# ethereum/pos-evolution

Measured on AMD Instinct MI355X. Metric: attestations aggregated/sec + get_head() p50 latency at 1M validators, higher is better.
Workload: dtype int32

## Files before the change

### pos_evolution_amd/csrc/engine_g1.cpp

```cpp
#include "engine_internal.h"

using namespace posevo;

namespace posevo {

void g1_stream_guard(pe_engine* h, hipStream_t s)
{
    if (h->side_ever && s != h->side_stream && s != h->fin_stream && s != h->norm_stream) (void)hipStreamWaitEvent(s, h->ev_join, 0);
}

int build_points30(pe_engine* h, uint64_t n)
{
    HIP_TRY(h, h->d_points30.ensure(std::max<size_t>(128, 4ull * G1_ROW_WORDS * n)));
    launch_g1_table_s30(h->stream, h->d_points.as<uint32_t>(), h->d_points30.as<uint32_t>(), n);
    HIP_TRY(h, hipGetLastError());
    h->points30_valid = true;
    return PE_OK;
}

int launch_g1_planned(pe_engine* h, const uint32_t* d_points, const uint32_t* d_members, const uint32_t* d_bits,
                      const G1Group* d_groups, const G1Plan& plan, uint8_t* d_out96, uint32_t* dev_jac,
                      hipStream_t s, hipStream_t fin, DevBuf* partials, DevBuf* lane_partials, const AttPlan* plan_dev,
                      const uint32_t* d_members1, uint64_t caller_rows, const G1Complement* cm)
{
    if (plan.n_groups == 0) return PE_OK;
    if (!s) s = h->stream;
    if (!fin) fin = s;
    if (!partials) partials = &h->d_partials;
    if (!lane_partials) lane_partials = &h->d_lane_partials;
    PE_TRY(ensure_quiesced(h, *partials,
                           std::max<size_t>(PE_G1_PARTIAL_BYTES, (size_t)PE_G1_PARTIAL_BYTES * plan.n_partials)));
    const size_t lane_bytes = (size_t)G1_LANE_PARTIAL_BYTES * G1_WG * ((plan.n_slots + G1_WG - 1) / G1_WG);
    PE_TRY(ensure_quiesced(h, *lane_partials, std::max<size_t>(PE_G1_PARTIAL_BYTES, lane_bytes)));
    const uint32_t* d_points30;
    if (d_points == h->d_points.as<uint32_t>()) {
        if (!h->points30_valid) return fail(h, PE_ERR_STATE, "the registry's table of the accumulation's field form was not built");
        d_points30 = h->d_points30.as<uint32_t>();
    } else {
        const uint64_t n_rows = caller_rows;
        if (d_points != h->d_tmp_points.as<uint32_t>() || 4ull * G1_ROW_WORDS * n_rows > h->d_tmp_points.cap)
            return fail(h, PE_ERR_STATE, "G1 sum over an unknown point table");
        HIP_TRY(h, h->d_tmp_points30.ensure(std::max<size_t>(128, 4ull * G1_ROW_WORDS * n_rows)));
        launch_g1_table_s30(s, d_points, h->d_tmp_points30.as<uint32_t>(), n_rows);
        d_points30 = h->d_tmp_points30.as<uint32_t>();
    }
    const bool chain = fin != s && fin == h->fin_stream;
    const int exclusive = chain && h->tune.exclusive && h->blocks.size() <= 4096 ? 1 : 0;
    const uint32_t sparse_max = cm && cm->info ? h->tune.g1_sparse_max() : 0u;
    const uint32_t* sparse_info = sparse_max ? cm->info : nullptr;
    if (sparse_max)
        launch_g1_absentees(s, d_points30, d_members, d_members1, d_bits, d_groups, plan.n_groups, plan_dev, cm->cmpl, sparse_info,
                            sparse_max, partials->as<uint32_t>());
    {
        const bool skip = !h->prof_timeline && s != h->stream && (h->acc_launches++ & 3) != 0;
        ProfScope ps(h, PE_KERNEL_G1_ACCUMULATE, s, skip);
        unsigned long long* clock_rec = nullptr;
        if (h->profiling) {
            if (!h->acc_clock && hipHostMalloc(reinterpret_cast<void**>(&h->acc_clock), 16ull * pe_engine::ACC_CLOCK_RING,
                                               hipHostMallocDefault) != hipSuccess) {
                (void)hipGetLastError();
                h->acc_clock = nullptr;
            }
            if (h->acc_clock) {
                clock_rec = h->acc_clock + 2 * (h->acc_clock_n++ % pe_engine::ACC_CLOCK_RING);
                clock_rec[0] = clock_rec[1] = 0;
            }
        }
        launch_g1_accumulate(s, d_points30, d_members, d_bits, d_groups, plan.n_groups, plan.n_slots,
                             lane_partials->as<uint32_t>(), partials->as<uint32_t>(), plan_dev, d_members1, exclusive, clock_rec,
                             cm ? cm->cmpl : nullptr, sparse_info, sparse_max);
    }
    hipStream_t ts = fin;
    if (ts != s) {
        HIP_TRY(h, hipEventRecord(h->ev_acc, s));
        HIP_TRY(h, hipStreamWaitEvent(ts, h->ev_acc, 0));
    }
    {
        ProfScope ps(h, PE_KERNEL_G1_TREE, ts);
        launch_g1_tree(ts, lane_partials->as<uint32_t>(), d_groups, plan.n_groups, plan.n_slots, partials->as<uint32_t>(),
                       ts != s ? 1 : 0,
                       plan_dev, exclusive, sparse_max ? cm->cmpl : nullptr, sparse_info, sparse_max);
    }
    hipStream_t ns = fin;
    if (chain && h->norm_stream) {
        ns = h->norm_stream;
        HIP_TRY(h, hipEventRecord(h->ev_tree, ts));
        HIP_TRY(h, hipStreamWaitEvent(ns, h->ev_tree, 0));
    } else if (ts != fin) {
        HIP_TRY(h, hipEventRecord(h->ev_tree, ts));
        HIP_TRY(h, hipStreamWaitEvent(fin, h->ev_tree, 0));
    }
    if (cm)
        for (int t = 0; t < 2; ++t)
            if (cm->ev[t]) HIP_TRY(h, hipStreamWaitEvent(ns, cm->ev[t], 0));
    {
        ProfScope ps(h, PE_KERNEL_G1_NORMALISE, ns);
        launch_g1_finish(ns, partials->as<uint32_t>(), d_groups, plan.n_groups, 0, 0, d_out96, dev_jac, plan_dev,
                         cm ? cm->cmpl : nullptr, cm ? cm->sums[0] : nullptr, cm ? cm->sums[1] : nullptr);
    }
    HIP_TRY(h, hipGetLastError());
    return PE_OK;
}

void committee_sums_drop(pe_engine* h)
{
    for (auto& t : h->tables) t.sums_valid = t.sums_wanted = false;
    if (h->sums_stream) (void)hipStreamSynchronize(h->sums_stream);
}
int build_committee_sums(pe_engine* h, CommitteeTable* t, bool defer)
{
    t->sums_valid = false;
    t->sums_wanted = false;
    if (!h->tune.committee_sums || !t->is_partition || !h->have_points || !h->points30_valid || h->dist_ready()) return PE_OK;
    if (t->n_committees == 0 || t->n_val_at_load != h->n_val || t->offsets.size() != (size_t)t->n_committees + 1) return PE_OK;
    const uint32_t C = t->n_committees;
    uint64_t total = t->offsets.back();
    uint32_t max_size = 0;
    for (uint32_t c = 0; c < C; ++c) max_size = std::max(max_size, t->offsets[c + 1] - t->offsets[c]);
    if (total == 0) return PE_OK;
    const uint32_t k = (uint32_t)std::max<uint64_t>({(uint64_t)G1_MIN_K, (total + G1_TARGET_LANES - 1) / G1_TARGET_LANES,
                                                     ((uint64_t)max_size + G1_WG - 1) / G1_WG});
    const uint32_t tasks = (max_size + k - 1) / k;
    uint32_t l2 = 0;
    while ((1u << l2) < tasks) ++l2;
    const uint64_t slots = (uint64_t)C << l2;
    if (slots > 4ull * G1_TARGET_LANES) return PE_OK;
    if (!h->sums_stream) {
        int least = 0, greatest = 0;
        HIP_TRY(h, hipDeviceGetStreamPriorityRange(&least, &greatest));
        HIP_TRY(h, hipStreamCreateWithPriority(&h->sums_stream, hipStreamNonBlocking, least));
    }
    hipStream_t ps = h->sums_stream;
    const size_t lane_bytes = (size_t)G1_LANE_PARTIAL_BYTES * G1_WG * ((slots + G1_WG - 1) / G1_WG);
    if (sizeof(G1Group) * (size_t)C > h->d_sum_groups.cap || lane_bytes > h->d_sum_lane.cap ||
        (size_t)PE_G1_PARTIAL_BYTES * C > t->d_sums.cap)
        HIP_TRY(h, hipStreamSynchronize(ps));
    HIP_TRY(h, h->d_sum_groups.ensure(sizeof(G1Group) * (size_t)C));
    HIP_TRY(h, h->d_sum_lane.ensure(lane_bytes));
    HIP_TRY(h, t->d_sums.ensure((size_t)PE_G1_PARTIAL_BYTES * C));
    if (defer) {
        t->sums_wanted = true;
        return PE_OK;
    }
    HIP_TRY(h, hipMemsetAsync(t->d_sums.p, 0, (size_t)PE_G1_PARTIAL_BYTES * C, ps));
    G1Group* d_groups = h->d_sum_groups.as<G1Group>();
    launch_g1_committee_groups(ps, t->d_offsets.as<uint32_t>(), C, k, l2, d_groups);
    launch_g1_accumulate(ps, h->d_points30.as<uint32_t>(), t->d_members.as<uint32_t>(), nullptr, d_groups, C, (uint32_t)slots,
                         h->d_sum_lane.as<uint32_t>(), t->d_sums.as<uint32_t>());
    launch_g1_tree(ps, h->d_sum_lane.as<uint32_t>(), d_groups, C, (uint32_t)slots, t->d_sums.as<uint32_t>());
    HIP_TRY(h, hipGetLastError());
    if (!t->ev_sums) HIP_TRY(h, hipEventCreateWithFlags(&t->ev_sums, hipEventDisableTiming));
    HIP_TRY(h, hipEventRecord(t->ev_sums, ps));
    t->sums_valid = true;
    return PE_OK;
}

int committee_sums_build_wanted(pe_engine* h, CommitteeTable* t)
{
    if (!t->sums_wanted || t->sums_valid || t->ready_pending) return PE_OK;
    if (t->ev_ready && hipEventQuery(t->ev_ready) != hipSuccess) { (void)hipGetLastError(); return PE_OK; }
    if (h->prep_stream && hipStreamQuery(h->prep_stream) != hipSuccess) { (void)hipGetLastError(); return PE_OK; }
    return build_committee_sums(h, t, false);
}

int sig_batch_flush(pe_engine* h)
{
    if (h->sig_batch.empty()) return PE_OK;
    std::vector<pe_engine::SigSeg> segs;
    segs.swap(h->sig_batch);
    const bool own = h->aux_stream && h->stream == h->own_stream;
    hipStream_t ss = own ? leg_stream(h) : h->stream;
    bool between = own && h->side_stream != nullptr;
    for (auto& sg : segs) between = between && sg.streaming;
    hipStream_t ds = between ? h->side_stream : ss;
    if (between) ss = ds;
    if (ss != h->stream) {
        HIP_TRY(h, hipEventRecord(h->ev_aux_fork, h->stream));
        HIP_TRY(h, hipStreamWaitEvent(ss, h->ev_aux_fork, 0));
        if (ds != ss) HIP_TRY(h, hipStreamWaitEvent(ds, h->ev_aux_fork, 0));
    }
    G2DecompressBatch b{};
    for (auto& sg : segs) {
        if (sg.copy_from) HIP_TRY(h, hipMemcpyAsync(const_cast<uint8_t*>(sg.d_in), sg.copy_from, sg.bytes, hipMemcpyDeviceToDevice, ds));
        if (sg.compressed) {
            b.in96[b.count] = sg.d_in;
            b.out_mont48[b.count] = sg.d_pts;
            b.status[b.count] = sg.d_status;
            b.n[b.count] = sg.n;
            ++b.count;
        } else {
            HIP_TRY(h, hipMemsetAsync(sg.d_status, 0, 4ull * sg.n, ds));
            launch_g2_convert(ds, sg.d_in, sg.d_pts, sg.n);
        }
    }
    if (b.count) {
        ProfScope ps(h, PE_KERNEL_G2_DECOMPRESS, ds);
        launch_g2_decompress_batch(ds, b);
    }
    if (ds != ss) {
        HIP_TRY(h, hipEventRecord(h->ev_sig, ds));
        HIP_TRY(h, hipStreamWaitEvent(ss, h->ev_sig, 0));
    }
    G2AggregateRowsBatch r{};
    for (auto& sg : segs) {
        if (sg.check_subgroup) launch_g2_subgroup_check(ss, sg.d_pts, sg.n, sg.d_status);
        r.pts[r.count] = sg.d_pts;
        r.status[r.count] = sg.d_status;
        r.ug[r.count] = sg.d_ug;
        r.member_row[r.count] = sg.d_member_row;
        r.plan_dev[r.count] = sg.plan_dev;
        r.out96[r.count] = sg.o_sig;
        r.out_bad[r.count] = sg.o_bad;
        r.n_groups[r.count] = sg.ng_bound;
        r.keep_mont48[r.count] = sg.keep_mont48;
        r.keep_bad[r.count] = sg.keep_bad;
        ++r.count;
    }
    {
        ProfScope ps(h, PE_KERNEL_G2_ACCUMULATE, ss);
        launch_g2_aggregate_rows(ss, r);
    }
    G2StatusOutBatch so{};
    for (auto& sg : segs) {
        so.src[so.count] = sg.d_status;
        so.dst_host[so.count] = sg.o_st;
        so.n[so.count] = sg.n;
        ++so.count;
    }
    launch_g2_status_out(ss, so);
    for (auto& sg : segs) {
        if (ss != h->stream) {
            pe_engine::PipeArena& a = h->arena[sg.arena];
            HIP_TRY(h, hipEventRecord(a.ev_leg, ss));
            a.leg_used = true;
        }
    }
    HIP_TRY(h, hipGetLastError());
    return PE_OK;
}
bool sig_batch_holds(const pe_engine* h, int arena)
{
    for (const auto& sg : h->sig_batch)
        if (sg.arena == arena) return true;
    return false;
}


int settle_signatures(pe_engine* h, const uint8_t* signatures96, uint64_t n, size_t tail_words, bool check_subgroup,
                      bool mark_identity, HostLap* lap, SettledSigs* out)
{
    hipStream_t s = h->stream;
// ... 544 lines not shown
```

### pos_evolution_amd/csrc/fp381_s30.h

```cpp
#pragma once
#include <stdint.h>

#include "pe_hd.h"

#ifndef PE_FQ30_ACC
#define PE_FQ30_ACC int64_t
#endif

namespace posevo {
namespace s30 {

constexpr int FQ_B = 30, FQ_N = 13;
constexpr int32_t FQ_MASK = (1 << FQ_B) - 1;

#include "fp381_s30_consts.inc"


using fq_acc = PE_FQ30_ACC;
PE_HD int32_t fq_digit32(int32_t v);
PE_HD int32_t fq_mont_digit(uint32_t v) { return fq_digit32((int32_t)v); }
PE_HD int32_t fq_carry32(int32_t v) { return (v >> FQ_B) + (int32_t)(((uint32_t)v >> (FQ_B - 1)) & 1u); }
PE_HD int32_t fq_norm_carry(int32_t v, int32_t) { return fq_carry32(v); }
PE_HD int32_t fq_p_carried(int i) { return FQ_P_CARRIED[i]; }

#include "fp381_lazy.inc"

PE_HD void fq_balance(fq& r, const fq& a)
{
    int32_t c = 0;
#pragma unroll
    for (int i = 0; i < FQ_N - 1; ++i) {
        const int32_t v = a.l[i] + c;
        r.l[i] = fq_digit32(v);
        c = fq_carry32(v);
    }
    r.l[FQ_N - 1] = a.l[FQ_N - 1] + c;
}
PE_HD void fq_from_mont32(fq& r, const uint32_t* w)
{
    fq a, an, k, t, c;
    fq_from_words32(a, w);
    fq_norm(an, a);
#pragma unroll
    for (int i = 0; i < FQ_N; ++i) k.l[i] = FQ_FROM_R32[i];
    fq_mul(t, an, k);
    fq_canonical_near(c, t);
    fq_balance(r, c);
}

}
}
```

### pos_evolution_amd/csrc/g1_kernels.hip

```cpp
#define POSEVO_FP_MUL_CALLED 1
#include <algorithm>
#include <hip/hip_ext.h>
#include "g1.h"
#include "g1_s30.h"
#include "fp_sqrt.h"
#include "kernels.h"
#include "wave64.h"

namespace posevo {

__global__ void __launch_bounds__(256) k_g1_convert(const uint8_t* __restrict__ be96, uint32_t* __restrict__ mont24,
                                                     uint64_t n)
{
    uint64_t i = (uint64_t)blockIdx.x * blockDim.x + threadIdx.x;
    if (i >= n) return;
    const uint8_t* src = be96 + 96 * i;
    uint32_t* dst = mont24 + (uint64_t)G1_ROW_WORDS * i;
    if (src[0] & 0x40) {
#pragma unroll
        for (int j = 0; j < 24; ++j) dst[j] = 0;
        return;
    }
    fp x, y, xm, ym;
    fp_load_be48(x, src);
// ... 694 lines not shown
        }
    }
    const bool gated = d.bits_word != NONE32;
    auto want = [&](uint32_t j, uint32_t& idx) -> bool {
        const uint32_t i = first + j;
        idx = members ? members[d.member_start + i] : d.member_start + i;
        if (!gated) return true;
        return (((bit_arena[d.bits_word + (i >> 5)] >> (i & 31)) & 1u) ^ invert) != 0;
    };
    auto fetch = [&](uint32_t j, fq& ox, fq& oy) -> bool {
        uint32_t idx;
        if (!want(j, idx)) return false;
        return load_point_s30(ox, oy, pts30, idx);
    };
    {
        fq qx, qy, nx, ny;
        bool have = false, nhave = false, w1 = false, w2 = false;
        uint32_t i1 = 0, i2 = 0;
        if (count > 0) {
            uint32_t i0;
            if (want(0, i0)) have = load_point_s30(qx, qy, pts30, i0);
        }
        if (count > 1) w1 = want(1, i1);
        for (uint32_t j = 0; j < count; ++j) {
            w2 = false;
            if (j + 2 < count) w2 = want(j + 2, i2);
            nhave = false;
            if (w1) nhave = load_point_s30(nx, ny, pts30, i1);
            if (have) {
                if (acc.inf) g1q_set_first(acc, qx, qy);
                else g1q_madd_fast(acc, qx, qy, exc);
            }
            qx = nx; qy = ny; have = nhave;
            i1 = i2; w1 = w2;
        }
    }
    G1_STAMP(1);
    G1_WAVE_END();
    if (exc) {
        g1q_set_inf(acc);
        for (uint32_t j = 0; j < count; ++j) {
            fq qx, qy;
            if (fetch(j, qx, qy)) g1q_add_affine<FqCalled>(acc, qx, qy, false);
        }
    }
    uint32_t* b = lane_partials + (size_t)blockIdx.x * G1S_WORDS * G1_WG + tid;
    const bool inf = acc.inf;
#pragma unroll
    for (int k = 0; k < FQ_N; ++k) {
        b[k * G1_WG] = inf ? 0u : (uint32_t)acc.x.l[k];
        b[(FQ_N + k) * G1_WG] = inf ? 0u : (uint32_t)acc.y.l[k];
        b[(2 * FQ_N + k) * G1_WG] = inf ? 0u : (uint32_t)acc.zz.l[k];
        b[(3 * FQ_N + k) * G1_WG] = inf ? 0u : (uint32_t)acc.zzz.l[k];
    }
    if (my_size == 1) {
        uint32_t* dst = wg_partials + (size_t)G1X_WORDS * my_out;
#pragma nounroll
        for (int c = 0; c < 4; ++c) {
            uint32_t w[12];
            fq_to_mont32_via<FqCalled>(w, acc.x);
#pragma unroll
            for (int k = 0; k < 12; ++k) dst[12 * c + k] = inf ? 0u : w[k];
            acc.x = acc.y;
            acc.y = acc.zz;
            acc.zz = acc.zzz;
        }
    }
    if (clock_rec && blockIdx.x == 0 && tid == 0) {
        clock_rec[0] = wall_clock64() - rec_w0;
        clock_rec[1] = clock64() - rec_c0;
    }
}
}

__global__ void __launch_bounds__(G1_WG) __attribute__((amdgpu_waves_per_eu(2, 2)))
k_g1_accumulate(const uint32_t* __restrict__ pts30, const uint32_t* __restrict__ members,
                const uint32_t* __restrict__ bit_arena, const G1Group* __restrict__ groups, uint32_t n_groups,
                uint32_t n_slots, uint32_t* __restrict__ lane_partials, uint32_t* __restrict__ wg_partials,
                const AttPlan* __restrict__ plan_dev, const uint32_t* __restrict__ members1,
                unsigned long long* __restrict__ clock_rec, const uint32_t* __restrict__ cmpl,
                const uint32_t* __restrict__ sparse_info, uint32_t sparse_max)
{
    s30::g1_accumulate_body(pts30, members, bit_arena, groups, n_groups, n_slots, lane_partials, wg_partials, plan_dev,
                            members1, clock_rec, cmpl, sparse_info, sparse_max);
}

void launch_g1_table_s30(hipStream_t s, const uint32_t* points_mont24, uint32_t* points_s30, uint64_t n)
{
    if (n == 0) return;
    hipLaunchKernelGGL(k_g1_table_s30, dim3((unsigned)((n + 255) / 256)), dim3(256), 0, s, points_mont24, points_s30, n);
}
void launch_g1_accumulate(hipStream_t s, const uint32_t* points_s30, const uint32_t* members,
                              const uint32_t* bit_arena, const G1Group* groups, uint32_t n_groups, uint32_t n_slots,
                              uint32_t* lane_partials, uint32_t* wg_partials48, const AttPlan* plan_dev,
                              const uint32_t* members1, int exclusive, unsigned long long* clock_rec, const uint32_t* cmpl,
                              const uint32_t* sparse_info, uint32_t sparse_max)
{
    if (n_groups == 0 || n_slots == 0) return;
    const unsigned blocks = (n_slots + G1_WG - 1) / G1_WG;
    size_t lds_bytes = 0;
    if (exclusive) {
        lds_bytes = G1_ACC_EXCLUSIVE_LDS;
        if (first_use_on_this_device<82>())
            (void)hipFuncSetAttribute(reinterpret_cast<const void*>(k_g1_accumulate), hipFuncAttributeMaxDynamicSharedMemorySize,
                                      (int)G1_ACC_EXCLUSIVE_LDS);
    }
    hipLaunchKernelGGL(k_g1_accumulate, dim3(blocks), dim3(G1_WG), lds_bytes, s, points_s30, members, bit_arena,
                       groups, n_groups, n_slots, lane_partials, wg_partials48, plan_dev, members1, clock_rec, cmpl, sparse_info,
                       sparse_max);
}

void launch_g1_tree(hipStream_t s, const uint32_t* lane_partials, const G1Group* groups, uint32_t n_groups,
                    uint32_t n_slots, uint32_t* wg_partials48, int one_per_cu, const AttPlan* plan_dev, int solo,
                    const uint32_t* cmpl, const uint32_t* sparse_info, uint32_t sparse_max)
{
    if (n_groups == 0 || n_slots == 0) return;
    const unsigned blocks = (n_slots + G1_WG - 1) / G1_WG;
    size_t lds_bytes = (s30::G1S_WORDS + 2) * G1_WG * sizeof(uint32_t);
    if (solo) {
        hipLaunchKernelGGL(k_g1_tree_solo, dim3(blocks), dim3(G1_WG), lds_bytes, s, lane_partials, groups, n_groups, n_slots,
                           wg_partials48, plan_dev, cmpl, sparse_info, sparse_max);
        return;
    }
    if (one_per_cu) {
        constexpr size_t padded = 84 * 1024;
        if (first_use_on_this_device<84>())
            (void)hipFuncSetAttribute(reinterpret_cast<const void*>(k_g1_tree), hipFuncAttributeMaxDynamicSharedMemorySize,
                                      (int)padded);
        lds_bytes = padded;
    }
    hipLaunchKernelGGL(k_g1_tree, dim3(blocks), dim3(G1_WG), lds_bytes, s, lane_partials, groups, n_groups, n_slots,
                       wg_partials48, plan_dev, cmpl, sparse_info, sparse_max);
}

namespace s30 {
__device__ __forceinline__ void g1q_from_lane_down(g1q& q, const g1q& p, int off)
{
#pragma unroll
    for (int j = 0; j < FQ_N; ++j) {
        q.x.l[j] = __shfl_down(p.x.l[j], off, 64);
        q.y.l[j] = __shfl_down(p.y.l[j], off, 64);
        q.zz.l[j] = __shfl_down(p.zz.l[j], off, 64);
        q.zzz.l[j] = __shfl_down(p.zzz.l[j], off, 64);
    }
    q.inf = __shfl_down((int)p.inf, off, 64) != 0;
    q.affine = false;
}
__device__ __forceinline__ void g1_absentees_body(const uint32_t* __restrict__ pts30, const uint32_t* __restrict__ members,
                                                  const uint32_t* __restrict__ members1,
                                                  const uint32_t* __restrict__ bit_arena, const G1Group* __restrict__ groups,
                                                  uint32_t n_groups, const AttPlan* __restrict__ plan_dev,
                                                  const uint32_t* __restrict__ cmpl,
                                                  const uint32_t* __restrict__ sparse_info, uint32_t sparse_max,
                                                  uint32_t* __restrict__ wg_partials)
{
    __shared__ uint32_t list[G1_SPARSE_CAP];
    if (plan_dev) n_groups = min(n_groups, plan_dev->n_groups);
    const uint32_t g = blockIdx.x;
    if (g >= n_groups) return;
    const G1Group d = groups[g];
    if (!g1_group_sparse(d, g, cmpl, sparse_info, sparse_max)) return;
    const uint32_t lane = threadIdx.x;
    const uint32_t n_words = (d.n_members + 31) >> 5;
    const uint32_t tail_mask = (d.n_members & 31) ? ((1u << (d.n_members & 31)) - 1u) : 0xFFFFFFFFu;
    uint32_t total = 0;
    for (uint32_t w0 = 0; w0 < n_words; w0 += 64) {
        const uint32_t w = w0 + lane;
        uint32_t absent = 0;
        if (w < n_words) absent = ~bit_arena[d.bits_word + w] & (w == n_words - 1 ? tail_mask : 0xFFFFFFFFu);
        const uint32_t mine = (uint32_t)__builtin_popcount(absent);
        uint32_t pos = total + wave_incl_scan(mine) - mine;
        while (absent) {
            if (pos < G1_SPARSE_CAP) list[pos] = 32u * w + (uint32_t)__builtin_ctz(absent);
            ++pos;
            absent &= absent - 1;
        }
        total += wave_sum(mine);
    }
    total = min(total, G1_SPARSE_CAP);
    __syncthreads();
    const uint32_t* __restrict__ mem = (d.k >> 31) ? members1 : members;
    g1q acc;
    g1q_set_inf(acc);
    for (uint32_t e = lane; e < total; e += 64) {
        const uint32_t i = list[e];
        const uint32_t idx = mem ? mem[d.member_start + i] : d.member_start + i;
        fq qx, qy;
        const bool have = load_point_s30(qx, qy, pts30, idx);
        g1q_add_affine<FqCalled>(acc, qx, qy, !have);
    }
    uint32_t live = min(total, 64u);
#pragma nounroll
    for (uint32_t off = 32; off >= 1; off >>= 1) {
        if (live <= off) continue;
        g1q q;
        g1q_from_lane_down(q, acc, (int)off);
        if (lane < off && lane + off < live) g1q_add<FqCalled>(acc, q);
        live = off;
    }
    fq coord;
#pragma unroll
    for (int j = 0; j < FQ_N; ++j) {
        const int32_t x = __shfl(acc.x.l[j], 0, 64), y = __shfl(acc.y.l[j], 0, 64);
        const int32_t zz = __shfl(acc.zz.l[j], 0, 64), zzz = __shfl(acc.zzz.l[j], 0, 64);
        coord.l[j] = lane == 0 ? x : lane == 1 ? y : lane == 2 ? zz : zzz;
    }
    const bool inf = __shfl((int)acc.inf, 0, 64) != 0;
    if (lane < 4) {
        uint32_t w[12];
        fq_to_mont32_via<FqCalled>(w, coord);
        uint4* dst = reinterpret_cast<uint4*>(wg_partials + (size_t)G1X_WORDS * d.out_base + 12 * lane);
        dst[0] = inf ? make_uint4(0, 0, 0, 0) : make_uint4(w[0], w[1], w[2], w[3]);
        dst[1] = inf ? make_uint4(0, 0, 0, 0) : make_uint4(w[4], w[5], w[6], w[7]);
        dst[2] = inf ? make_uint4(0, 0, 0, 0) : make_uint4(w[8], w[9], w[10], w[11]);
    }
}
}

__global__ void __launch_bounds__(64) __attribute__((amdgpu_waves_per_eu(2, 8)))
k_g1_absentees(const uint32_t* __restrict__ pts30, const uint32_t* __restrict__ members,
               const uint32_t* __restrict__ members1, const uint32_t* __restrict__ bit_arena,
               const G1Group* __restrict__ groups, uint32_t n_groups, const AttPlan* __restrict__ plan_dev,
               const uint32_t* __restrict__ cmpl, const uint32_t* __restrict__ sparse_info, uint32_t sparse_max,
               uint32_t* __restrict__ wg_partials)
{
    s30::g1_absentees_body(pts30, members, members1, bit_arena, groups, n_groups, plan_dev, cmpl, sparse_info, sparse_max,
                           wg_partials);
}

void launch_g1_absentees(hipStream_t s, const uint32_t* points_s30, const uint32_t* members, const uint32_t* members1,
                         const uint32_t* bit_arena, const G1Group* groups, uint32_t n_groups, const AttPlan* plan_dev,
                         const uint32_t* cmpl, const uint32_t* sparse_info, uint32_t sparse_max, uint32_t* wg_partials48)
{
    if (n_groups == 0 || !cmpl || !sparse_info || sparse_max == 0) return;
    hipLaunchKernelGGL(k_g1_absentees, dim3(n_groups), dim3(64), 0, s, points_s30, members, members1, bit_arena, groups,
                       n_groups, plan_dev, cmpl, sparse_info, sparse_max, wg_partials48);
}

__global__ void __launch_bounds__(64)
k_g1_finish(const uint32_t* __restrict__ partials, const G1Group* __restrict__ groups, uint32_t n_groups,
            uint32_t n_parts_fixed, uint32_t part_stride, uint8_t* __restrict__ out_be96,
            uint32_t* __restrict__ out_jac, const AttPlan* __restrict__ plan_dev, const uint32_t* __restrict__ cmpl,
            const uint32_t* __restrict__ sums0, const uint32_t* __restrict__ sums1)
{
    if (plan_dev) n_groups = min(n_groups, plan_dev->n_groups);
    const uint32_t g = blockIdx.x * blockDim.x + threadIdx.x;
    if (g >= n_groups) return;
    uint32_t first, n_parts, stride;
    if (groups) {
        const G1Group d = groups[g];
        first = d.out_base;
        n_parts = d.log2_block > 8 ? (d.n_tasks + G1_WG - 1) / G1_WG : 1u;
        if (d.n_tasks == 0) n_parts = 0;
        stride = 1;
    } else {
        first = g;
        n_parts = n_parts_fixed;
        stride = part_stride;
    }
    const uint32_t verdict = cmpl ? cmpl[g] : NONE32;
    const uint32_t* csum = nullptr;
    if (verdict != NONE32) csum = ((verdict >> 31) ? sums1 : sums0) + (size_t)G1X_WORDS * (verdict & 0x7FFFFFFFu);
    g1x acc;
    g1x_set_inf(acc);
    for (uint32_t k = 0; k < n_parts + (csum ? 1u : 0u); ++k) {
        g1x q;
        const uint32_t* src = partials + (size_t)G1X_WORDS * (first + (uint64_t)k * stride);
        if (k == n_parts) {
            fp ny;
            fp_neg(ny, acc.y);
            acc.y = ny;
            src = csum;
        }
        global_load_x(q, src);
        g1x_add(acc, q);
    }
    if (out_jac) global_store_x(out_jac + (size_t)G1X_WORDS * g, acc);
    if (!out_be96) return;
    uint8_t* o = out_be96 + 96ull * g;
    uint32_t* ow = reinterpret_cast<uint32_t*>(o);
    if (g1x_is_inf(acc)) {
#pragma unroll
        for (int j = 0; j < 24; ++j) ow[j] = 0;
        o[0] = 0x40;
        return;
    }
    fp x, y;
    g1x_to_affine_plain(x, y, acc);
    fp_store_be48(o, x);
    fp_store_be48(o + 48, y);
}

void launch_g1_finish(hipStream_t s, const uint32_t* partials48, const G1Group* groups, uint32_t n_groups,
                      uint32_t n_parts_fixed, uint32_t part_stride, uint8_t* out_be96, uint32_t* out_xyzz48,
                      const AttPlan* plan_dev, const uint32_t* cmpl, const uint32_t* sums0, const uint32_t* sums1)
{
    if (n_groups == 0) return;
    hipLaunchKernelGGL(k_g1_finish, dim3((n_groups + 63) / 64), dim3(64), 0, s, partials48, groups, n_groups,
                       n_parts_fixed, part_stride, out_be96, out_xyzz48, plan_dev, cmpl, sums0, sums1);
}

__global__ void __launch_bounds__(256)
k_g1_committee_groups(const uint32_t* __restrict__ offsets, uint32_t n_committees, uint32_t k, uint32_t log2_block,
                      G1Group* __restrict__ groups)
{
    const uint32_t c = blockIdx.x * 256 + threadIdx.x;
    if (c >= n_committees) return;
    G1Group d;
    d.member_start = offsets[c];
    d.n_members = offsets[c + 1] - offsets[c];
    d.bits_word = NONE32;
    d.slot_base = c << log2_block;
    d.n_tasks = (d.n_members + k - 1) / k;
    d.k = k;
    d.log2_block = log2_block;
    d.out_base = c;
    groups[c] = d;
}
void launch_g1_committee_groups(hipStream_t s, const uint32_t* offsets, uint32_t n_committees, uint32_t k, uint32_t log2_block,
                                G1Group* groups)
{
    if (n_committees == 0) return;
    hipLaunchKernelGGL(k_g1_committee_groups, dim3((n_committees + 255) / 256), dim3(256), 0, s, offsets, n_committees, k,
                       log2_block, groups);
}

}
```

### pos_evolution_amd/csrc/kernels.h

```cpp
#pragma once
#include <hip/hip_runtime.h>
#include <stdint.h>

namespace posevo {

template <int TAG>
static bool first_use_on_this_device()
{
    static bool done[64] = {false};
    int dev = 0;
    (void)hipGetDevice(&dev);
    if (dev < 0 || dev >= 64) return true;
    if (done[dev]) return false;
    done[dev] = true;
    return true;
}

constexpr uint32_t NONE32 = 0xFFFFFFFFu;
constexpr int G1_ROW_WORDS = 32;
constexpr int G2_WG_SLOTS = 128;
constexpr int G1_WG = 256;
constexpr int G1_LANE_PARTIAL_BYTES = 208;
constexpr int TREE_MAX_BLOCKS = 8192;
constexpr int VOTES_MAX_WG = 256;

struct G1Group {
    uint32_t member_start;
    uint32_t n_members;
    uint32_t bits_word;
    uint32_t slot_base;
    uint32_t n_tasks;
    uint32_t k;
    uint32_t log2_block;
    uint32_t out_base;
};

void launch_g1_convert(hipStream_t s, const uint8_t* be96, uint32_t* mont24, uint64_t n);
void launch_g1_table_s30(hipStream_t s, const uint32_t* points_mont24, uint32_t* points_s30, uint64_t n);
struct AttPlan;
void launch_g1_accumulate(hipStream_t s, const uint32_t* points_s30, const uint32_t* members,
                          const uint32_t* bit_arena, const G1Group* groups, uint32_t n_groups, uint32_t n_slots,
                          uint32_t* lane_partials, uint32_t* wg_partials48, const AttPlan* plan_dev = nullptr,
                          const uint32_t* members1 = nullptr, int exclusive = 0, unsigned long long* clock_rec = nullptr,
                          const uint32_t* cmpl = nullptr, const uint32_t* sparse_info = nullptr, uint32_t sparse_max = 0);
void launch_g1_committee_groups(hipStream_t s, const uint32_t* offsets, uint32_t n_committees, uint32_t k, uint32_t log2_block,
                                G1Group* groups);
constexpr uint32_t G1_SPARSE_MAX = 128;
constexpr uint32_t G1_SPARSE_CAP = 256;
void launch_g1_absentees(hipStream_t s, const uint32_t* points_s30, const uint32_t* members, const uint32_t* members1,
                         const uint32_t* bit_arena, const G1Group* groups, uint32_t n_groups, const AttPlan* plan_dev,
                         const uint32_t* cmpl, const uint32_t* sparse_info, uint32_t sparse_max, uint32_t* wg_partials48);
constexpr size_t G1_ACC_EXCLUSIVE_LDS = 82 * 1024;
void launch_g1_tree(hipStream_t s, const uint32_t* lane_partials, const G1Group* groups, uint32_t n_groups,
                    uint32_t n_slots, uint32_t* wg_partials48, int one_per_cu = 0, const AttPlan* plan_dev = nullptr,
                    int solo = 0, const uint32_t* cmpl = nullptr, const uint32_t* sparse_info = nullptr,
                    uint32_t sparse_max = 0);
void launch_g1_finish(hipStream_t s, const uint32_t* partials48, const G1Group* groups, uint32_t n_groups,
                      uint32_t n_parts_fixed, uint32_t part_stride, uint8_t* out_be96, uint32_t* out_xyzz48,
                      const AttPlan* plan_dev = nullptr, const uint32_t* cmpl = nullptr, const uint32_t* sums0 = nullptr,
                      const uint32_t* sums1 = nullptr);

struct TreeDev {
    const uint32_t* size;
    const uint32_t* parent;
    const uint32_t* rank;
    const uint8_t* leaf_ok;
    const uint32_t* pos_of_idx;
    const uint32_t* idx_of_pos;
    uint32_t n;
};
struct VoteTotals {
    unsigned long long total_active_balance;
    unsigned long long num_active;
};

struct AttRow {
    uint32_t member_base;
    uint32_t n_bits;
    uint32_t bits_word;
    uint32_t block_idx;
    uint32_t epoch_p1;
    uint32_t order;
    uint32_t flag_mask;
    uint32_t which;
    uint32_t slot;
    uint32_t gate;
};
__host__ __device__ inline AttRow att_row_fork_choice(uint32_t member_base, uint32_t n_bits, uint32_t bits_word, uint32_t block_idx,
                                                      uint64_t target_epoch, uint64_t slot, uint32_t order, uint32_t gate)
{
    return AttRow{member_base, n_bits, bits_word, block_idx, (uint32_t)target_epoch + 1, order, 0u, 0u, (uint32_t)slot, gate};
}
__host__ __device__ inline AttRow att_row_flags(uint32_t member_base, uint32_t n_bits, uint32_t bits_word, uint32_t flag_mask,
                                                uint32_t which, uint32_t order, uint32_t gate)
{
    return AttRow{member_base, n_bits, bits_word, 0u, 0u, order, flag_mask, which, 0u, gate};
}
void launch_lmd_update(hipStream_t s, const AttRow* rows, uint32_t n_rows, const uint32_t* members,
                       const uint32_t* bit_arena, const uint8_t* flags, uint64_t* vote_key, uint32_t* vote_block,
                       uint32_t* vote_slot = nullptr, const uint32_t* gates = nullptr);
void launch_invert_committees(hipStream_t s, const uint32_t* members, const uint32_t* offsets, uint32_t n_committees,
                              uint32_t* inv_comm, uint32_t* inv_pos, uint64_t n_val);
void launch_lmd_validator_major(hipStream_t s, const AttRow* rows, const uint32_t* crow_start,
                                const uint32_t* crow_list, const uint32_t* inv_comm, const uint32_t* inv_pos,
                                const uint32_t* bit_arena, const uint8_t* flags, uint64_t n_val, uint64_t* vote_key,
                                uint32_t* vote_block, uint32_t* vote_slot = nullptr, const uint32_t* gates = nullptr);
void launch_participation(hipStream_t s, const AttRow* rows, uint32_t n_rows, const uint32_t* members,
                          const uint32_t* bit_arena, const uint16_t* eff_increments,
                          uint64_t base_reward_per_increment, uint32_t* part_cur_words,
                          uint32_t* part_prev_words, uint64_t* numerators, const uint32_t* numerator_slot,
                          const uint32_t* gates = nullptr);
struct UnionGroup {
    uint32_t list_start;
    uint32_t n_atts;
    uint32_t n_bits;
    uint32_t out_word;
};

constexpr uint32_t ATT_EMPTY = 0xFFFFFFFFu;
struct TableDev {
    uint64_t epoch;
    const uint32_t* members;
    const uint32_t* offsets;
    const uint32_t* inv_comm;
    const uint32_t* inv_pos;
    uint32_t n_committees;
    uint32_t valid;
};
struct TablesDev {
    TableDev t[2];
    uint64_t slots_per_epoch;
};
struct AttPlan {
    uint32_t n_groups;
    uint32_t n_slots;
    uint32_t k, log2_block;
    uint32_t out_words, out_bytes;
    uint32_t error;
    uint32_t packed_same;
    uint32_t n_rows_table[2];
    uint32_t n_rows_in;
    uint32_t last_error;
    unsigned long long total_members;
};
struct AttGroup {
    uint32_t rep;
    uint32_t n_atts, list_start, cursor;
    uint32_t n_bits, out_word, out_byte;
    uint32_t table;
    uint32_t pos, size, member_base;
    uint32_t sig_valid;
    uint32_t status_agg;
    uint32_t index_over;
    uint32_t pad[2];
};
struct BlockTableDev {
    const uint32_t* root_tab;
    uint32_t root_mask;
    const uint8_t* roots;
    const unsigned long long* slot_pos;
    const uint32_t* parent_pos;
    const uint32_t* pos_of_idx;
    uint32_t n_blocks;
};
struct FcCtx {
    unsigned long long cur_slot, cur_epoch, prev_epoch, slots_per_epoch;
};
struct StateCtxDev {
    unsigned long long slot, cur_epoch, prev_epoch, slots_per_epoch, min_inclusion_delay, sqrt_spe;
    unsigned long long cj_epoch, pj_epoch;
    uint8_t cj_root[32], pj_root[32];
    uint32_t tgt_blk[2];
    uint32_t head_blk[64];
    unsigned long long base_reward_per_increment;
};
struct PlanSync {
    uint32_t ticket;
    uint32_t max_size;
    uint32_t rows_t[2];
    uint32_t mis_key;
    uint32_t err;
    uint32_t pad[2];
    unsigned long long total_members, pad2[3];
};
struct PlanRec {
    unsigned long long agg[3], incl[3], pad[2];
};
constexpr uint32_t PLAN_WG = 256;
constexpr uint32_t PLAN_MAX_ROWS = 1u << 24;
struct AttPlanArgs {
    const void* rows; uint32_t n; const uint32_t* n_dev;
    const uint32_t* tab; const uint32_t* cnt_tab; const uint32_t* slot_of;
    uint32_t* rep_of; uint32_t* gid_of_row;
    AttGroup* grp; UnionGroup* ug;
    uint32_t* crow_start[2]; uint32_t* crow_cursor[2]; uint32_t* crow_cnt[2];
    PlanSync* sync; PlanRec* rec;
    AttPlan* plan; AttPlan* plan_host;
    uint64_t out_arena_cap; uint32_t target_slots, slot_cap, min_k, want_pk;
    TablesDev tables;
};
void launch_att_plan(hipStream_t s, const AttPlanArgs& a);
void launch_att_pack(hipStream_t s, const void* rows, const AttGroup* grp, const AttPlan* plan, const uint32_t* res_bits,
                     const uint32_t* res_info, uint32_t slots, uint32_t wps, uint32_t* send);
void launch_att_unpack(hipStream_t s, const uint32_t* recv, uint32_t world, uint32_t slots, uint32_t wps, void* out_rows,
                       uint32_t* out_bits, uint32_t* n_dev, uint32_t* err_host);
void launch_att_validate_state(hipStream_t s, const void* rows, const AttGroup* grp, const AttPlan* plan, uint32_t n_bound,
                               uint32_t cap, BlockTableDev bt, const StateCtxDev& st, const uint32_t* union_info,
                               AttRow* out_rows, int32_t* status_dev, int32_t* status_host, uint32_t* err_host);
void launch_participation_tables(hipStream_t s, const AttRow* rows, TablesDev tables, uint32_t* const crow_start[2],
                                 uint32_t* const crow_list[2], const AttPlan* plan, const uint32_t* bit_arena,
                                 const uint16_t* eff_increments, uint64_t base_reward_per_increment,
                                 uint32_t* part_cur_words, uint32_t* part_prev_words, uint64_t* numerators,
                                 const uint32_t* gates, uint32_t cap);
// ... 317 lines not shown
```

Measured before the change: 6.946 billion.

## Fold committee-sum combination for sparse groups into the absentees kernel

For groups on the sparse-absentee path, the absentees kernel now loads the precomputed committee sum, converts it to the s30 form, and adds it to the negated absentee accumulation itself. It uses a four-lane quad add staged through LDS, with a single-lane fallback. The finish kernel then skips the committee-sum add for those groups, so it no longer does a serial per-thread point add with a Montgomery conversion. In exchange, the absentees launch must now wait on the committee-sum events and does extra work plus several barriers per group.

```diff
diff --git a/pos_evolution_amd/csrc/engine_g1.cpp b/pos_evolution_amd/csrc/engine_g1.cpp
--- a/pos_evolution_amd/csrc/engine_g1.cpp
+++ b/pos_evolution_amd/csrc/engine_g1.cpp
@@ -48,9 +48,12 @@
     const int exclusive = chain && h->tune.exclusive && h->blocks.size() <= 4096 ? 1 : 0;
     const uint32_t sparse_max = cm && cm->info ? h->tune.g1_sparse_max() : 0u;
     const uint32_t* sparse_info = sparse_max ? cm->info : nullptr;
-    if (sparse_max)
+    if (sparse_max) {
+        for (int t = 0; t < 2; ++t)
+            if (cm->ev[t]) HIP_TRY(h, hipStreamWaitEvent(s, cm->ev[t], 0));
         launch_g1_absentees(s, d_points30, d_members, d_members1, d_bits, d_groups, plan.n_groups, plan_dev, cm->cmpl, sparse_info,
-                            sparse_max, partials->as<uint32_t>());
+                            sparse_max, cm->sums[0], cm->sums[1], partials->as<uint32_t>());
+    }
     {
         const bool skip = !h->prof_timeline && s != h->stream && (h->acc_launches++ & 3) != 0;
         ProfScope ps(h, PE_KERNEL_G1_ACCUMULATE, s, skip);
@@ -96,7 +99,8 @@
     {
         ProfScope ps(h, PE_KERNEL_G1_NORMALISE, ns);
         launch_g1_finish(ns, partials->as<uint32_t>(), d_groups, plan.n_groups, 0, 0, d_out96, dev_jac, plan_dev,
-                         cm ? cm->cmpl : nullptr, cm ? cm->sums[0] : nullptr, cm ? cm->sums[1] : nullptr);
+                         cm ? cm->cmpl : nullptr, cm ? cm->sums[0] : nullptr, cm ? cm->sums[1] : nullptr, sparse_info,
+                         sparse_max);
     }
     HIP_TRY(h, hipGetLastError());
     return PE_OK;
diff --git a/pos_evolution_amd/csrc/fp381_s30.h b/pos_evolution_amd/csrc/fp381_s30.h
--- a/pos_evolution_amd/csrc/fp381_s30.h
+++ b/pos_evolution_amd/csrc/fp381_s30.h
@@ -36,17 +36,21 @@
     }
     r.l[FQ_N - 1] = a.l[FQ_N - 1] + c;
 }
-PE_HD void fq_from_mont32(fq& r, const uint32_t* w)
+struct FqHere {
+    PE_HD_MEMBER void mul(fq& r, const fq& a, const fq& b) { fq_mul(r, a, b); }
+};
+template <class MP> PE_HD void fq_from_mont32_via(fq& r, const uint32_t* w)
 {
     fq a, an, k, t, c;
     fq_from_words32(a, w);
     fq_norm(an, a);
 #pragma unroll
     for (int i = 0; i < FQ_N; ++i) k.l[i] = FQ_FROM_R32[i];
-    fq_mul(t, an, k);
+    MP::mul(t, an, k);
     fq_canonical_near(c, t);
     fq_balance(r, c);
 }
+PE_HD void fq_from_mont32(fq& r, const uint32_t* w) { fq_from_mont32_via<FqHere>(r, w); }
 
 }
 }
diff --git a/pos_evolution_amd/csrc/g1_kernels.hip b/pos_evolution_amd/csrc/g1_kernels.hip
--- a/pos_evolution_amd/csrc/g1_kernels.hip
+++ b/pos_evolution_amd/csrc/g1_kernels.hip
@@ -870,6 +870,7 @@
                                                   uint32_t n_groups, const AttPlan* __restrict__ plan_dev,
                                                   const uint32_t* __restrict__ cmpl,
                                                   const uint32_t* __restrict__ sparse_info, uint32_t sparse_max,
+                                                  const uint32_t* __restrict__ sums0, const uint32_t* __restrict__ sums1,
                                                   uint32_t* __restrict__ wg_partials)
 {
     __shared__ uint32_t list[G1_SPARSE_CAP];
@@ -916,14 +917,89 @@
         if (lane < off && lane + off < live) g1q_add<FqCalled>(acc, q);
         live = off;
     }
+    static_assert(12 * FQ_N + 1 <= (int)G1_SPARSE_CAP, "the index list's LDS holds three points and a flag");
+    {
+        const uint32_t verdict = cmpl[g];
+        const uint32_t* csum = ((verdict >> 31) ? sums1 : sums0) + (size_t)G1X_WORDS * (verdict & 0x7FFFFFFFu);
+        fq sc;
+        fq_set_zero(sc);
+        if (lane < 4) {
+            const uint4* src = reinterpret_cast<const uint4*>(csum + 12 * lane);
+            const uint4 v0 = src[0], v1 = src[1], v2 = src[2];
+            const uint32_t w[12] = {v0.x, v0.y, v0.z, v0.w, v1.x, v1.y, v1.z, v1.w, v2.x, v2.y, v2.z, v2.w};
+            fq_from_mont32_via<FqCalled>(sc, w);
+        }
+        const bool n_inf = __shfl((int)acc.inf, 0, 64) != 0;
+        const bool s_inf = __shfl((int)fq_limbs_zero(sc), 2, 64) != 0;
+        __syncthreads();
+        if (lane == 0) {
+#pragma unroll
+            for (int j = 0; j < FQ_N; ++j) {
+                list[j] = (uint32_t)acc.x.l[j];
+                list[FQ_N + j] = (uint32_t)-acc.y.l[j];
+                list[2 * FQ_N + j] = (uint32_t)acc.zz.l[j];
+                list[3 * FQ_N + j] = (uint32_t)acc.zzz.l[j];
+            }
+            list[12 * FQ_N] = n_inf && s_inf ? 1u : 0u;
+        }
+        if (lane < 4) {
+#pragma unroll
+            for (int j = 0; j < FQ_N; ++j) list[(4 + lane) * FQ_N + j] = (uint32_t)sc.l[j];
+        }
+        __syncthreads();
+        bool done = false;
+        if (!n_inf && !s_inf) {
+            const int q4 = (int)(lane & 3);
+            const int ia = q4 == 0 ? 0 : q4 == 1 ? 4 : q4 == 2 ? 1 : 5, ib = q4 == 0 ? 6 : q4 == 1 ? 2 : q4 == 2 ? 7 : 3;
+            fq a, b, oa, ob;
+#pragma unroll
+            for (int j = 0; j < FQ_N; ++j) {
+                a.l[j] = (int32_t)list[ia * FQ_N + j];
+                b.l[j] = (int32_t)list[ib * FQ_N + j];
+            }
+            done = g1s_add_quad(oa, ob, q4, a, b);
+            if (done && lane >= 1 && lane < 4) {
+                const int io = lane == 2 ? 8 : lane == 1 ? 10 : 11;
+#pragma unroll
+                for (int j = 0; j < FQ_N; ++j) {
+                    list[io * FQ_N + j] = (uint32_t)oa.l[j];
+                    if (lane == 2) list[9 * FQ_N + j] = (uint32_t)ob.l[j];
+                }
+            }
+        }
+        if (!done && lane == 0) {
+            g1q p, q;
+#pragma unroll
+            for (int j = 0; j < FQ_N; ++j) {
+                p.x.l[j] = (int32_t)list[j];
+                p.y.l[j] = (int32_t)list[FQ_N + j];
+                p.zz.l[j] = (int32_t)list[2 * FQ_N + j];
+                p.zzz.l[j] = (int32_t)list[3 * FQ_N + j];
+                q.x.l[j] = (int32_t)list[4 * FQ_N + j];
+                q.y.l[j] = (int32_t)list[5 * FQ_N + j];
+                q.zz.l[j] = (int32_t)list[6 * FQ_N + j];
+                q.zzz.l[j] = (int32_t)list[7 * FQ_N + j];
+            }
+            p.inf = n_inf;
+            p.affine = false;
+            q.inf = s_inf;
+            q.affine = false;
+            g1q_add<FqCalled>(p, q);
+#pragma unroll
+            for (int j = 0; j < FQ_N; ++j) {
+                list[8 * FQ_N + j] = (uint32_t)p.x.l[j];
+                list[9 * FQ_N + j] = (uint32_t)p.y.l[j];
+                list[10 * FQ_N + j] = (uint32_t)p.zz.l[j];
+                list[11 * FQ_N + j] = (uint32_t)p.zzz.l[j];
+            }
+            list[12 * FQ_N] = p.inf ? 1u : 0u;
+        }
+        __syncthreads();
+    }
     fq coord;
 #pragma unroll
-    for (int j = 0; j < FQ_N; ++j) {
-        const int32_t x = __shfl(acc.x.l[j], 0, 64), y = __shfl(acc.y.l[j], 0, 64);
-        const int32_t zz = __shfl(acc.zz.l[j], 0, 64), zzz = __shfl(acc.zzz.l[j], 0, 64);
-        coord.l[j] = lane == 0 ? x : lane == 1 ? y : lane == 2 ? zz : zzz;
-    }
-    const bool inf = __shfl((int)acc.inf, 0, 64) != 0;
+    for (int j = 0; j < FQ_N; ++j) coord.l[j] = (int32_t)list[(8 + (lane & 3)) * FQ_N + j];
+    const bool inf = list[12 * FQ_N] != 0;
     if (lane < 4) {
         uint32_t w[12];
         fq_to_mont32_via<FqCalled>(w, coord);
@@ -940,43 +1016,47 @@
                const uint32_t* __restrict__ members1, const uint32_t* __restrict__ bit_arena,
                const G1Group* __restrict__ groups, uint32_t n_groups, const AttPlan* __restrict__ plan_dev,
                const uint32_t* __restrict__ cmpl, const uint32_t* __restrict__ sparse_info, uint32_t sparse_max,
-               uint32_t* __restrict__ wg_partials)
+               const uint32_t* __restrict__ sums0, const uint32_t* __restrict__ sums1, uint32_t* __restrict__ wg_partials)
 {
     s30::g1_absentees_body(pts30, members, members1, bit_arena, groups, n_groups, plan_dev, cmpl, sparse_info, sparse_max,
-                           wg_partials);
+                           sums0, sums1, wg_partials);
 }
 
 void launch_g1_absentees(hipStream_t s, const uint32_t* points_s30, const uint32_t* members, const uint32_t* members1,
                          const uint32_t* bit_arena, const G1Group* groups, uint32_t n_groups, const AttPlan* plan_dev,
-                         const uint32_t* cmpl, const uint32_t* sparse_info, uint32_t sparse_max, uint32_t* wg_partials48)
+                         const uint32_t* cmpl, const uint32_t* sparse_info, uint32_t sparse_max, const uint32_t* sums0,
+                         const uint32_t* sums1, uint32_t* wg_partials48)
 {
     if (n_groups == 0 || !cmpl || !sparse_info || sparse_max == 0) return;
     hipLaunchKernelGGL(k_g1_absentees, dim3(n_groups), dim3(64), 0, s, points_s30, members, members1, bit_arena, groups,
-                       n_groups, plan_dev, cmpl, sparse_info, sparse_max, wg_partials48);
+                       n_groups, plan_dev, cmpl, sparse_info, sparse_max, sums0, sums1, wg_partials48);
 }
 
 __global__ void __launch_bounds__(64)
 k_g1_finish(const uint32_t* __restrict__ partials, const G1Group* __restrict__ groups, uint32_t n_groups,
             uint32_t n_parts_fixed, uint32_t part_stride, uint8_t* __restrict__ out_be96,
             uint32_t* __restrict__ out_jac, const AttPlan* __restrict__ plan_dev, const uint32_t* __restrict__ cmpl,
-            const uint32_t* __restrict__ sums0, const uint32_t* __restrict__ sums1)
+            const uint32_t* __restrict__ sums0, const uint32_t* __restrict__ sums1,
+            const uint32_t* __restrict__ sparse_info, uint32_t sparse_max)
 {
     if (plan_dev) n_groups = min(n_groups, plan_dev->n_groups);
     const uint32_t g = blockIdx.x * blockDim.x + threadIdx.x;
     if (g >= n_groups) return;
     uint32_t first, n_parts, stride;
+    bool sparse = false;
     if (groups) {
         const G1Group d = groups[g];
         first = d.out_base;
         n_parts = d.log2_block > 8 ? (d.n_tasks + G1_WG - 1) / G1_WG : 1u;
         if (d.n_tasks == 0) n_parts = 0;
         stride = 1;
+        sparse = g1_group_sparse(d, g, cmpl, sparse_info, sparse_max);
     } else {
         first = g;
         n_parts = n_parts_fixed;
         stride = part_stride;
     }
-    const uint32_t verdict = cmpl ? cmpl[g] : NONE32;
+    const uint32_t verdict = cmpl && !sparse ? cmpl[g] : NONE32;
     const uint32_t* csum = nullptr;
     if (verdict != NONE32) csum = ((verdict >> 31) ? sums1 : sums0) + (size_t)G1X_WORDS * (verdict & 0x7FFFFFFFu);
     g1x acc;
@@ -1011,11 +1091,13 @@
 
 void launch_g1_finish(hipStream_t s, const uint32_t* partials48, const G1Group* groups, uint32_t n_groups,
                       uint32_t n_parts_fixed, uint32_t part_stride, uint8_t* out_be96, uint32_t* out_xyzz48,
-                      const AttPlan* plan_dev, const uint32_t* cmpl, const uint32_t* sums0, const uint32_t* sums1)
+                      const AttPlan* plan_dev, const uint32_t* cmpl, const uint32_t* sums0, const uint32_t* sums1,
+                      const uint32_t* sparse_info, uint32_t sparse_max)
 {
     if (n_groups == 0) return;
     hipLaunchKernelGGL(k_g1_finish, dim3((n_groups + 63) / 64), dim3(64), 0, s, partials48, groups, n_groups,
-                       n_parts_fixed, part_stride, out_be96, out_xyzz48, plan_dev, cmpl, sums0, sums1);
+                       n_parts_fixed, part_stride, out_be96, out_xyzz48, plan_dev, cmpl, sums0, sums1, sparse_info,
+                       sparse_max);
 }
 
 __global__ void __launch_bounds__(256)
diff --git a/pos_evolution_amd/csrc/kernels.h b/pos_evolution_amd/csrc/kernels.h
--- a/pos_evolution_amd/csrc/kernels.h
+++ b/pos_evolution_amd/csrc/kernels.h
@@ -49,7 +49,8 @@
 constexpr uint32_t G1_SPARSE_CAP = 256;
 void launch_g1_absentees(hipStream_t s, const uint32_t* points_s30, const uint32_t* members, const uint32_t* members1,
                          const uint32_t* bit_arena, const G1Group* groups, uint32_t n_groups, const AttPlan* plan_dev,
-                         const uint32_t* cmpl, const uint32_t* sparse_info, uint32_t sparse_max, uint32_t* wg_partials48);
+                         const uint32_t* cmpl, const uint32_t* sparse_info, uint32_t sparse_max, const uint32_t* sums0,
+                         const uint32_t* sums1, uint32_t* wg_partials48);
 constexpr size_t G1_ACC_EXCLUSIVE_LDS = 82 * 1024;
 void launch_g1_tree(hipStream_t s, const uint32_t* lane_partials, const G1Group* groups, uint32_t n_groups,
                     uint32_t n_slots, uint32_t* wg_partials48, int one_per_cu = 0, const AttPlan* plan_dev = nullptr,
@@ -58,7 +59,7 @@
 void launch_g1_finish(hipStream_t s, const uint32_t* partials48, const G1Group* groups, uint32_t n_groups,
                       uint32_t n_parts_fixed, uint32_t part_stride, uint8_t* out_be96, uint32_t* out_xyzz48,
                       const AttPlan* plan_dev = nullptr, const uint32_t* cmpl = nullptr, const uint32_t* sums0 = nullptr,
-                      const uint32_t* sums1 = nullptr);
+                      const uint32_t* sums1 = nullptr, const uint32_t* sparse_info = nullptr, uint32_t sparse_max = 0);
 
 struct TreeDev {
     const uint32_t* size;
```

After: 6.287 billion. -9.5%, worse.
